# atunnd/Hair-centric-Image-Retrieval

Measured on AMD Instinct MI355X. Metric: query-images/sec (embed+top-10) ViT-B/16 vs 1M gallery, 1/2/4/8 GPU, higher is better.
Workload: dtype f16; 1 GPU; ViT-B/16 (HSimCLR ViTWrapper, random init) embed + top-10 over 1000000 x 768 f32 gallery row-sharded over 1 GPU(s); query_batch_per_gpu=880, global_query_batch=880, gallery_rows=1000000, gallery_dtype=f32, topk=10, sim_mode=filtered, residual_stream=f16, steps_in_flight=2, parallelism=gallery-shard1+query-dp1

## Files before the change

### hair-centric-image-retrieval_amd/csrc/gemm.hip

```cpp
#include "sim_core.h"
#include "act.h"
#include "gemm_plan.h"
#include "patch_plan.h"
#include "gemm_stage_addr.h"
#include <stdlib.h>

namespace {

using GemmCfg = SimCfg<_Float16, 2, 2, 2>;

constexpr int EPI_RESID_F16_STATS = 7;
constexpr int EPI_LN_BIAS_F16 = 8;
constexpr int EPI_LN_BIAS_GELU_F16 = 9;
constexpr int EPI_BIAS_F16_DUAL_GELU = 10;
constexpr int EPI_PATCH_F16_STATS = 11;

struct GemmArgs {
  const _Float16* a;
  const _Float16* w;
  const float* bias;
  const float* scale;
  void* out;
  int64_t m, lda, ldw, ldo;
  int n, k;
  const float* ln_stats;
  const float* ln_c1;
  float* stats_part;
  const void* resid;
  void* out2;
  int64_t stats_ld = 0;
};

__device__ __forceinline__ int xcd_remap(int bid, int nwg) { return gemm_xcd_remap(bid, nwg); }

template <int EPI, int NTILES>
__device__ __forceinline__ void gemm_epilogue_t(const GemmArgs& g, const f32x16 (&acc)[NTILES][2],
                                                int64_t m0, int nbase, int wave_m, int lane) {
  const int r = lane & 31, h = lane >> 5;
#pragma unroll
  for (int mt = 0; mt < 2; ++mt) {
    const int64_t m = m0 + wave_m * 64 + mt * 32 + r;
    if (m >= g.m) continue;
#pragma unroll
    for (int nt = 0; nt < NTILES; ++nt) {
#pragma unroll
      for (int grp = 0; grp < 4; ++grp) {
        const int n = nbase + nt * 32 + 8 * grp + 4 * h;
        if (n >= g.n) continue;
        f32x4 v;
#pragma unroll
        for (int e = 0; e < 4; ++e) v[e] = acc[nt][mt][4 * grp + e];
        f32x4 b = {0.f, 0.f, 0.f, 0.f};
        if (g.bias) b = *reinterpret_cast<const f32x4*>(g.bias + n);
        if constexpr (EPI == HCIR_EPI_AFFINE_RELU_F16 || EPI == HCIR_EPI_AFFINE_F32) {
          const f32x4 s = *reinterpret_cast<const f32x4*>(g.scale + n);
#pragma unroll
          for (int e = 0; e < 4; ++e) v[e] = __builtin_fmaf(v[e], s[e], b[e]);
        } else {
#pragma unroll
          for (int e = 0; e < 4; ++e) v[e] += b[e];
        }
        if constexpr (EPI == HCIR_EPI_BIAS_F16 || EPI == HCIR_EPI_BIAS_GELU_F16 ||
                      EPI == HCIR_EPI_AFFINE_RELU_F16) {
          f16x4 o;
#pragma unroll
          for (int e = 0; e < 4; ++e) {
            float x = v[e];
            if constexpr (EPI == HCIR_EPI_BIAS_GELU_F16) x = gelu_erf(x);
            if constexpr (EPI == HCIR_EPI_AFFINE_RELU_F16) x = fmaxf(x, 0.f);
            o[e] = (_Float16)x;
          }
          *reinterpret_cast<f16x4*>(static_cast<_Float16*>(g.out) + m * g.ldo + n) = o;
        } else if constexpr (EPI == HCIR_EPI_BIAS_RESID_F16) {
          _Float16* p = static_cast<_Float16*>(g.out) + m * g.ldo + n;
          const f16x4 oh = *reinterpret_cast<const f16x4*>(static_cast<const _Float16*>(g.resid) + m * g.ldo + n);
          f16x4 o;
#pragma unroll
          for (int e = 0; e < 4; ++e) {
            const float sc1 = g.scale ? g.scale[n + e] : 1.0f;
            o[e] = (_Float16)__builtin_fmaf(sc1, v[e], (float)oh[e]);
          }
          *reinterpret_cast<f16x4*>(p) = o;
        } else if constexpr (EPI == HCIR_EPI_BIAS_RESID_F32) {
          float* p = static_cast<float*>(g.out) + m * g.ldo + n;
          f32x4 o = *reinterpret_cast<const f32x4*>(static_cast<const float*>(g.resid) + m * g.ldo + n);
          if (g.scale) {
            const f32x4 s = *reinterpret_cast<const f32x4*>(g.scale + n);
#pragma unroll
            for (int e = 0; e < 4; ++e) o[e] = __builtin_fmaf(s[e], v[e], o[e]);
          } else {
#pragma unroll
            for (int e = 0; e < 4; ++e) o[e] += v[e];
          }
          *reinterpret_cast<f32x4*>(p) = o;
        } else {
          *reinterpret_cast<f32x4*>(static_cast<float*>(g.out) + m * g.ldo + n) = v;
        }
      }
    }
  }
}

template <int EPI>
__device__ __forceinline__ void gemm_epilogue(const GemmArgs& g, const f32x16 (&acc)[2][2],
                                              int64_t m0, int n0, int wave_n, int wave_m, int lane) {
  gemm_epilogue_t<EPI, 2>(g, acc, m0, n0 + wave_n * 64, wave_m, lane);
}
__device__ __forceinline__ void launder(f32x4& v) { asm volatile("" : "+v"(v)); }

struct WaveAcc {
  f32x4 a[8][4];
  __device__ __forceinline__ void zero() {
#pragma unroll
    for (int x = 0; x < 8; ++x)
#pragma unroll
      for (int y = 0; y < 4; ++y)
#pragma unroll
        for (int i = 0; i < 4; ++i) a[x][y][i] = 0.f;
  }
};

__device__ __forceinline__ float sum8_dpp(float v) {
  v += __builtin_bit_cast(float, __builtin_amdgcn_update_dpp(0, __builtin_bit_cast(int, v), 0xB1, 0xF, 0xF, true));
  v += __builtin_bit_cast(float, __builtin_amdgcn_update_dpp(0, __builtin_bit_cast(int, v), 0x4E, 0xF, 0xF, true));
  v += __builtin_bit_cast(float, __builtin_amdgcn_update_dpp(0, __builtin_bit_cast(int, v), 0x141, 0xF, 0xF, true));
  return v;
}

__device__ __forceinline__ f32x2 slice_stats8(const f16x8& o) {
  float xv[8], s1 = 0.f;
#pragma unroll
  for (int e = 0; e < 8; ++e) {
    xv[e] = (float)o[e];
    s1 += xv[e];
  }
  const float mean_s = sum8_dpp(s1) * (1.0f / 64.0f);
  float m2 = 0.f;
#pragma unroll
  for (int e = 0; e < 8; ++e) {
    const float dv = xv[e] - mean_s;
    m2 = __builtin_fmaf(dv, dv, m2);
  }
  return (f32x2){mean_s, sum8_dpp(m2)};
}

struct PatchRowMap {
  int mb, bi0, rem0, np;
  float inv;
  __device__ __forceinline__ PatchRowMap() : mb(0), bi0(0), rem0(0), np(1), inv(1.f) {}
  __device__ __forceinline__ PatchRowMap(int64_t m0w, int64_t mtot, int np_) : np(np_) {
    mb = (int)(m0w < mtot ? m0w : mtot - 1);
    bi0 = mb / np;
    rem0 = mb - bi0 * np;
    inv = 1.0f / (float)np;
  }
  __device__ __forceinline__ void map(int64_t m, int64_t mtot, int& bi, int& pi) const {
    const int r = rem0 + ((int)(m < mtot ? m : mtot - 1) - mb);
    int q = (int)((float)r * inv);
    q += ((q + 1) * np <= r) ? 1 : 0;
    q -= (q * np > r) ? 1 : 0;
    bi = bi0 + q;
    pi = r - q * np;
  }
};

template <int EPI, bool FULL, int NTW, int MTT, int MTH, class GA>
__device__ __forceinline__ void gemm_epilogue_lds_impl(const GA& g, const f32x4 (&acc)[NTW][MTT], int mt0,
                                                       char* region, int64_t m0w, int nbase, int lane) {
  constexpr bool kLn = (EPI == EPI_LN_BIAS_F16 || EPI == EPI_LN_BIAS_GELU_F16);
  constexpr bool kGelu = (EPI == HCIR_EPI_BIAS_GELU_F16 || EPI == EPI_LN_BIAS_GELU_F16);
  constexpr bool kResidH = (EPI == HCIR_EPI_BIAS_RESID_F16 || EPI == EPI_RESID_F16_STATS);
  constexpr bool kDual = (EPI == EPI_BIAS_F16_DUAL_GELU);
  constexpr bool kPatch = (EPI == EPI_PATCH_F16_STATS);
  constexpr bool kF16 = (EPI == HCIR_EPI_BIAS_F16 || kGelu || kLn ||
                         EPI == HCIR_EPI_AFFINE_RELU_F16 || kResidH || kDual || kPatch);
  constexpr bool kAffine = (EPI == HCIR_EPI_AFFINE_RELU_F16 || EPI == HCIR_EPI_AFFINE_F32);
  constexpr int FPP = kF16 ? 64 : 32;
  constexpr int NPASS = NTW * 16 / FPP;
  constexpr int NIT = MTH * 2;
  constexpr int UB = (NIT % 4 == 0) ? 4 : 3;
  static_assert(NIT % UB == 0 && (NTW * 16) % FPP == 0, "geometry");
  const int rrow = lane >> 3, rchunk = lane & 7;

  constexpr bool kScaleA = kF16 && (EPI == HCIR_EPI_AFFINE_RELU_F16 || kResidH);
  f32x4 biasA[kF16 ? NTW : 1], scaleA[kScaleA ? NTW : 1];
  bool has_scale = false;
  if constexpr (kF16) {
    has_scale = kScaleA && (EPI == HCIR_EPI_AFFINE_RELU_F16 || g.scale != nullptr);
#pragma unroll
    for (int t = 0; t < NTW; ++t) {
      const int n = nbase + 16 * t + 4 * (lane >> 4);
      biasA[t] = (f32x4){0.f, 0.f, 0.f, 0.f};
      if (g.bias) biasA[t] = *reinterpret_cast<const f32x4*>(g.bias + n);
      if constexpr (kScaleA) {
        scaleA[t] = (f32x4){1.f, 1.f, 1.f, 1.f};
        if (has_scale) scaleA[t] = *reinterpret_cast<const f32x4*>(g.scale + n);
      }
    }
  }
  constexpr int NB = kF16 ? 2 : 1;
  f32x4 bias[NPASS][NB], scale[NPASS][NB];
#pragma unroll
  for (int pass = 0; pass < NPASS; ++pass) {
    if constexpr (kF16) break;
#pragma unroll
    for (int j = 0; j < NB; ++j) {
      const int n = nbase + pass * FPP + rchunk * (kF16 ? 8 : 4) + 4 * j;
      bias[pass][j] = (f32x4){0.f, 0.f, 0.f, 0.f};
      scale[pass][j] = (f32x4){1.f, 1.f, 1.f, 1.f};
      if (g.bias) bias[pass][j] = *reinterpret_cast<const f32x4*>(g.bias + n);
      if (kAffine || (EPI == HCIR_EPI_BIAS_RESID_F32 && g.scale))
        scale[pass][j] = *reinterpret_cast<const f32x4*>(g.scale + n);
    }
  }
  float ln_rs[MTH], ln_mean[MTH];
  f32x4 c1a[NTW];
  if constexpr (kLn) {
#pragma unroll
    for (int mt = 0; mt < MTH; ++mt) {
      int64_t mm = m0w + 16 * mt + (lane & 15);
      mm = mm < g.m ? mm : g.m - 1;
      ln_mean[mt] = g.ln_stats[2 * mm];
      ln_rs[mt] = g.ln_stats[2 * mm + 1];
    }
#pragma unroll
    for (int t = 0; t < NTW; ++t) c1a[t] = *reinterpret_cast<const f32x4*>(g.ln_c1 + nbase + 16 * t + 4 * (lane >> 4));
  }
  PatchRowMap rm;
  if constexpr (kPatch) rm = PatchRowMap(m0w, g.m, g.np);
  asm volatile("s_waitcnt vmcnt(0)" ::: "memory");
  if constexpr (kLn) {
#pragma unroll
    for (int mt = 0; mt < MTH; ++mt) asm volatile("" : "+v"(ln_rs[mt]));
#pragma unroll
    for (int mt = 0; mt < MTH; ++mt) asm volatile("" : "+v"(ln_mean[mt]));
#pragma unroll
    for (int t = 0; t < NTW; ++t) launder(c1a[t]);
  }
  if constexpr (kF16) {
#pragma unroll
    for (int t = 0; t < NTW; ++t) {
      launder(biasA[t]);
      if constexpr (kScaleA) launder(scaleA[t]);
    }
  } else {
#pragma unroll
    for (int pass = 0; pass < NPASS; ++pass)
#pragma unroll
      for (int j = 0; j < NB; ++j) {
        launder(bias[pass][j]);
        launder(scale[pass][j]);
      }
  }

  constexpr int NITER = kDual ? 2 * NPASS : NPASS;
#pragma unroll
  for (int iter = 0; iter < NITER; ++iter) {
    const int pass = kDual ? iter >> 1 : iter;
    const bool second = kDual && (iter & 1);
    const int r16 = lane & 15, q16 = lane >> 4;
#pragma unroll
    for (int mt = 0; mt < MTH; ++mt) {
      const int row = mt * 16 + r16;
      if constexpr (kF16) {
        f32x4 posA[kPatch ? 4 : 1];
        if constexpr (kPatch) {
          int bi, pi;
          rm.map(m0w + row, g.m, bi, pi);
          const float* prow = g.pos + (int64_t)(1 + pi) * g.n + nbase + 64 * pass + 4 * q16;
#pragma unroll
          for (int q = 0; q < 4; ++q) posA[q] = *reinterpret_cast<const f32x4*>(prow + 16 * q);
        }
#pragma unroll
        for (int q = 0; q < 4; ++q) {
          const int nt = 4 * pass + q;
          f16x4 o;
          float xs[4];
#pragma unroll
          for (int e = 0; e < 4; ++e) {
            float x = acc[nt][mt0 + mt][e];
            const float bb = biasA[nt][e];
            if constexpr (kLn) {
              x = __builtin_fmaf(ln_rs[mt], __builtin_fmaf(-ln_mean[mt], c1a[nt][e], x), bb);
            } else if constexpr (EPI == HCIR_EPI_AFFINE_RELU_F16) {
              x = fmaxf(__builtin_fmaf(x, scaleA[nt][e], bb), 0.f);
            } else if constexpr (kResidH) {
              x = scaleA[nt][e] * (x + bb);
            } else if constexpr (kPatch) {
              x = __builtin_fmaf(g.pos_mult, posA[q][e], x + bb);
            } else {
              x += bb;
            }
            xs[e] = x;
          }
          if (kGelu || second) {
#pragma unroll
            for (int e = 0; e < 4; e += 2) {
              const gelu_f32x2 y = gelu_erf2((gelu_f32x2){xs[e], xs[e + 1]});
              xs[e] = y[0];
              xs[e + 1] = y[1];
            }
          }
#pragma unroll
          for (int e = 0; e < 4; ++e) o[e] = (_Float16)xs[e];
          const int chunk = 2 * q + (q16 >> 1);
          *reinterpret_cast<f16x4*>(region + row * 128 + ((chunk ^ (row & 7)) << 4) + 8 * (q16 & 1)) = o;
        }
      } else {
#pragma unroll
        for (int q = 0; q < 2; ++q) {
          const int nt = 2 * pass + q;
          const int chunk = 4 * q + q16;
          *reinterpret_cast<f32x4*>(region + row * 128 + ((chunk ^ (row & 7)) << 4)) = acc[nt][mt0 + mt];
        }
      }
    }
    if constexpr (kF16) {
      const int n = nbase + pass * 64 + rchunk * 8;
#pragma unroll
      for (int it0 = 0; it0 < NIT; it0 += UB) {
        f16x8 oldh[UB];
        if constexpr (kResidH) {
#pragma unroll
          for (int u = 0; u < UB; ++u) {
            const int64_t mm = m0w + (it0 + u) * 8 + rrow;
#pragma unroll
            for (int e = 0; e < 8; ++e) oldh[u][e] = (_Float16)0.f;
            if (FULL || mm < g.m)
              oldh[u] = *reinterpret_cast<const f16x8*>(static_cast<const _Float16*>(g.resid) + mm * g.ldo + n);
          }
        }
#pragma unroll
        for (int u = 0; u < UB; ++u) {
          const int row = (it0 + u) * 8 + rrow;
          const f16x8 v = *reinterpret_cast<const f16x8*>(region + row * 128 + ((rchunk ^ (row & 7)) << 4));
          f16x8 o;
          if constexpr (kResidH)
            o = v + oldh[u];
          else
            o = v;
          int64_t m = m0w + row;
          const int64_t mrow = m;
          if constexpr (kPatch) {
            int bi, pi;
            rm.map(m, g.m, bi, pi);
            m = (int64_t)bi * (g.np + 1) + 1 + pi;
          }
          if (FULL || mrow < g.m)
            __builtin_nontemporal_store(
                o, reinterpret_cast<f16x8*>(static_cast<_Float16*>(second ? g.out2 : g.out) + m * g.ldo + n));
          if constexpr (EPI == EPI_RESID_F16_STATS || kPatch) {
            const f32x2 ss = slice_stats8(o);
            if (rchunk == 0 && (FULL || mrow < g.m) && (!kPatch || g.stats_part)) {
              const int64_t slice = (nbase >> 6) + pass;
              *reinterpret_cast<f32x2*>(g.stats_part + (slice * (g.stats_ld ? g.stats_ld : g.m) + m) * 2) = ss;
            }
          }
        }
      }
    } else {
      const int n = nbase + pass * 32 + rchunk * 4;
      const f32x4 b = bias[pass][0], sc = scale[pass][0];
#pragma unroll
      for (int it0 = 0; it0 < NIT; it0 += UB) {
        f32x4 oldv[UB];
#pragma unroll
        for (int u = 0; u < UB; ++u) {
          const int64_t mm = m0w + (it0 + u) * 8 + rrow;
          oldv[u] = (f32x4){0.f, 0.f, 0.f, 0.f};
          if constexpr (EPI == HCIR_EPI_BIAS_RESID_F32) {
            if (FULL || mm < g.m)
              oldv[u] = *reinterpret_cast<const f32x4*>(static_cast<const float*>(g.resid) + mm * g.ldo + n);
          }
        }
#pragma unroll
        for (int u = 0; u < UB; ++u) {
          const int row = (it0 + u) * 8 + rrow;
          const int64_t mm = m0w + row;
          f32x4 v = *reinterpret_cast<const f32x4*>(region + row * 128 + ((rchunk ^ (row & 7)) << 4));
          if constexpr (EPI == HCIR_EPI_AFFINE_F32) {
#pragma unroll
            for (int e = 0; e < 4; ++e) v[e] = __builtin_fmaf(v[e], sc[e], b[e]);
          } else if constexpr (EPI == HCIR_EPI_BIAS_RESID_F32) {
#pragma unroll
            for (int e = 0; e < 4; ++e) v[e] = __builtin_fmaf(sc[e], v[e] + b[e], oldv[u][e]);
          } else {
#pragma unroll
            for (int e = 0; e < 4; ++e) v[e] += b[e];
          }
          if (FULL || mm < g.m) *reinterpret_cast<f32x4*>(static_cast<float*>(g.out) + mm * g.ldo + n) = v;
        }
      }
    }
  }
}

template <int EPI, int NTW, int MTT, int MTH, class GA>
__device__ __forceinline__ void gemm_epilogue_lds(const GA& g, const f32x4 (&acc)[NTW][MTT], int mt0,
                                                  char* region, int64_t m0w, int nbase, int lane) {
  asm volatile("" : "+v"(lane));
  if (m0w + 16 * MTH <= g.m)
    gemm_epilogue_lds_impl<EPI, true, NTW, MTT, MTH>(g, acc, mt0, region, m0w, nbase, lane);
  else
    gemm_epilogue_lds_impl<EPI, false, NTW, MTT, MTH>(g, acc, mt0, region, m0w, nbase, lane);
}

template <int EPI, bool GLDS>
__global__ __launch_bounds__(256, 2) void gemm_f16_kernel(GemmArgs g, int tiles_n, int tiles_m) {
  using Cfg = GemmCfg;
  __shared__ __attribute__((aligned(16))) char lds[Cfg::LDS_BYTES];
  const int tid = threadIdx.x, lane = tid & 63, wave = tid >> 6;
  const int wave_n = wave >> 1, wave_m = wave & 1;
  const int t = xcd_remap(blockIdx.x, tiles_n * tiles_m);
  const int tn = t % tiles_n, tm = t / tiles_n;
  const int n0 = tn * 128;
  const int64_t m0 = (int64_t)tm * 128;
  const int nkc = (g.k + 63) / 64;

  f32x16 acc[2][2];
#pragma unroll
  for (int a = 0; a < 2; ++a)
#pragma unroll
    for (int b = 0; b < 2; ++b)
#pragma unroll
      for (int i = 0; i < 16; ++i) acc[a][b][i] = 0.f;

  if constexpr (GLDS) {
    sim_stage_glds<_Float16, Cfg>(lds, g.w, n0, g.n - 1, g.a, m0, g.m - 1, g.k, 0, tid);
    for (int kc = 0; kc < nkc; ++kc) {
      const int cur = kc & 1;
      sim_glds_retire_and_sync();
      if (kc + 1 < nkc)
        sim_stage_glds<_Float16, Cfg>(lds + (cur ^ 1) * Cfg::STAGE_BYTES, g.w, n0, g.n - 1, g.a, m0,
                                      g.m - 1, g.k, kc + 1, tid);
      sim_stage_mfma<_Float16, Cfg, 2>(acc, lds + cur * Cfg::STAGE_BYTES, wave_n, wave_m, lane);
    }
  } else {
    u32x4 regs[Cfg::NLOAD];
    sim_stage_load<_Float16, Cfg>(regs, g.w, n0, g.n - 1, g.a, m0, g.m - 1, g.k, 0, tid);
    sim_stage_store<Cfg>(regs, lds, tid);
    __syncthreads();
    for (int kc = 0; kc < nkc; ++kc) {
      const int cur = kc & 1;
      if (kc + 1 < nkc)
        sim_stage_load<_Float16, Cfg>(regs, g.w, n0, g.n - 1, g.a, m0, g.m - 1, g.k, kc + 1, tid);
      sim_stage_mfma<_Float16, Cfg, 2>(acc, lds + cur * Cfg::STAGE_BYTES, wave_n, wave_m, lane);
      if (kc + 1 < nkc) sim_stage_store<Cfg>(regs, lds + (cur ^ 1) * Cfg::STAGE_BYTES, tid);
      __syncthreads();
    }
  }
  gemm_epilogue<EPI>(g, acc, m0, n0, wave_n, wave_m, lane);
}

#ifdef HCIR_DIAG_GSTAMPS
__device__ unsigned long long g_gemm_stamps[256 * 8];
#define HCIR_GSTAMP(cond, i)                                                                   \
  do {                                                                                         \
    if ((cond) && threadIdx.x == 0 && blockIdx.x < 256)                                        \
      g_gemm_stamps[blockIdx.x * 8 + (i)] = __builtin_amdgcn_s_memrealtime();                  \
  } while (0)
#else
#define HCIR_GSTAMP(cond, i) \
  do {                       \
  } while (0)
#endif


struct G256 {
  static constexpr int NT = 512;
  static constexpr int TN = 256, TM = 256;
  static constexpr int WAVES_N = 2, WAVES_M = 4;
  static constexpr int ROWS = TN + TM;
  static constexpr int STAGE_BYTES = ROWS * 128;
  static constexpr int NLOAD = ROWS * 8 / NT;
  static constexpr int NW = TN * 8 / NT;
  static constexpr bool N_GROUPED = true;
  static_assert(WAVES_N * WAVES_M * 64 == NT && NT * NW == TN * 8, "geometry");
};

struct GMid {
  static constexpr int NT = 256;
  static constexpr int TN = 128, TM = 192;
  static constexpr int WAVES_N = 2, WAVES_M = 2;
  static constexpr int ROWS = TN + TM;
  static constexpr int STAGE_BYTES = ROWS * 128;
  static constexpr int NLOAD = ROWS * 8 / NT;
  static constexpr int NW = TN * 8 / NT;
  static constexpr bool N_GROUPED = false;
  static_assert(WAVES_N * WAVES_M * 64 == NT && NT * NW == TN * 8, "geometry");
};

template <class G>
struct GemmStages {
  int issue_kc = 0, issue_ti = 0;
  const char* wbase = nullptr;
  const char* abase = nullptr;
  int a_last = 0;
  GemmTileOrigins org;
  const GemmArgs& g;
  char* const lds;
  const int tiles_n, tiles_m, tid;
  const int ntiles = tiles_n * tiles_m;
  const int nkc = g.k / 64;
  const int my_tiles =
      (int)blockIdx.x < ntiles ? (ntiles - (int)blockIdx.x + (int)gridDim.x - 1) / (int)gridDim.x : 0;
  const int nsteps = my_tiles * nkc;
  const int wave_dst = __builtin_amdgcn_readfirstlane((tid & ~63) * 16);
  uint32_t woff, aoff;

  __device__ __forceinline__ GemmStages(const GemmArgs& g_, char* lds_, int tiles_n_, int tiles_m_, int tid_)
      : g(g_), lds(lds_), tiles_n(tiles_n_), tiles_m(tiles_m_), tid(tid_) {
    set_lane_offsets();
  }

  __device__ __forceinline__ void set_lane_offsets() {
    int otid = tid;
    asm volatile("" : "+v"(otid));
    woff = gemm_lane_off(otid, g.ldw);
    aoff = gemm_lane_off(otid, g.lda);
  }

  __device__ __forceinline__ void tile_origin(int ti, int& n0, int64_t& m0) const {
    gemm_tile_origin<G::N_GROUPED, G::TN, G::TM>((int)blockIdx.x, (int)gridDim.x, ti, tiles_n, tiles_m, n0, m0);
  }

  __device__ __forceinline__ void origin(int ti, int& n0, int64_t& m0) const {
    int mt;
    org.get(issue_ti - ti, n0, mt);
    m0 = (int64_t)mt * G::TM;
  }

  __device__ __forceinline__ void next_tile() {
    org.shift();
    if (issue_ti < my_tiles) {
      int n0;
      int64_t m0;
      tile_origin(issue_ti, n0, m0);
      org.set(n0, (int)(m0 / G::TM));
      wbase = reinterpret_cast<const char*>(g.w + (int64_t)n0 * g.ldw);
      abase = reinterpret_cast<const char*>(g.a + m0 * g.lda);
      a_last = gemm_tile_last_row<G::TM>(g.m, m0);
    }
  }

  __device__ __forceinline__ bool ragged() const { return a_last < G::TM - 1; }

  template <bool RAGGED>
  __device__ __forceinline__ void issue_piece_as(int slot, int i) const {
    const uint32_t dst = lds_addr(lds) + slot * G::STAGE_BYTES + wave_dst + G::NT * i * 16;
    int otid = tid;
    if constexpr (RAGGED) asm volatile("" : "+v"(otid));
    int64_t base;
    uint32_t off;
// ... 376 lines not shown
    const int bfirst = (int)m0 / g.np;
    ibase = reinterpret_cast<const char*>(g.img + (int64_t)bfirst * g.c * g.h * g.w_px);
#pragma unroll
    for (int i = 0; i < NA; ++i) {
      int64_t m = m0 + (otid >> 3) + 64 * i;
      m = m < g.m ? m : g.m - 1;
      const int mi = (int)m;
      const int bi = mi / g.np, pi = mi - bi * g.np;
      const int py = pi / g.gw, px = pi - py * g.gw;
      aoff[i] = (uint32_t)((((bi - bfirst) * g.c * g.h + py * 16 + (chunk >> 1)) * g.w_px + px * 16 + 8 * (chunk & 1)) * 4);
    }
  };
  f32x4 stage_a[2 * NA];
  auto gather_load = [&](int kc) {
    const char* kbase = ibase + ((int64_t)(kc >> 2) * g.h + 4 * (kc & 3)) * g.w_px * 4;
#pragma unroll
    for (int i = 0; i < NA; ++i) {
      stage_a[2 * i] = *reinterpret_cast<const f32x4*>(kbase + aoff[i]);
      stage_a[2 * i + 1] = *reinterpret_cast<const f32x4*>(kbase + aoff[i] + 16);
    }
  };
  auto gather_store = [&](int slot) {
#pragma unroll
    for (int i = 0; i < NA; ++i) {
      f16x8 v;
#pragma unroll
      for (int e = 0; e < 4; ++e) {
        v[e] = (_Float16)stage_a[2 * i][e];
        v[4 + e] = (_Float16)stage_a[2 * i + 1][e];
      }
      *reinterpret_cast<f16x8*>(lds + slot * G256::STAGE_BYTES + sim_slot_off(G256::TN + (tid >> 3) + 64 * i, tid & 7)) = v;
    }
  };

  WaveAcc acc;
  acc.zero();

  if (nsteps > 0) {
    stg.next_tile();
    set_rows(0);
    gather_load(0);
#pragma unroll
    for (int i = 0; i < G256::NW; ++i) stg.issue_piece(0, i);
    gather_store(0);
    stg.issue_advance();
    if (stg.issue_kc == 0 && stg.issue_ti < stg.my_tiles) set_rows(stg.issue_ti);
  }

  int kc = 0, ti = 0;
  for (int step = 0; step < nsteps; ++step) {
    asm volatile("s_waitcnt vmcnt(0) lgkmcnt(0)" ::: "memory");
    __builtin_amdgcn_s_barrier();

    const char* st = lds + (step & 1) * G256::STAGE_BYTES;
    const bool do_issue = step + 1 < nsteps;
    const int islot = (step + 1) & 1;
    const int r16 = lane & 15, kq = lane >> 4;
    if (do_issue) gather_load(stg.issue_kc);
#pragma unroll
    for (int ks2 = 0; ks2 < 2; ++ks2) {
      const int chunk = 4 * ks2 + kq;
      u32x4 bf[4];
#pragma unroll
      for (int mt = 0; mt < 4; ++mt)
        bf[mt] = *reinterpret_cast<const u32x4*>(st + sim_slot_off(G256::TN + wave_m * 64 + mt * 16 + r16, chunk));
#pragma unroll
      for (int half = 0; half < 2; ++half) {
        u32x4 af[4];
#pragma unroll
        for (int q = 0; q < 4; ++q)
          af[q] = *reinterpret_cast<const u32x4*>(
              st + sim_slot_off(wave_n * 128 + (4 * half + q) * 16 + r16, chunk));
        if (do_issue && ks2 == 0 && half == 0) {
#pragma unroll
          for (int i = 0; i < G256::NW; ++i) stg.issue_piece(islot, i);
        }
#pragma unroll
        for (int q = 0; q < 4; ++q)
#pragma unroll
          for (int mt = 0; mt < 4; ++mt)
            acc.a[4 * half + q][mt] = __builtin_amdgcn_mfma_f32_16x16x32_f16(
                __builtin_bit_cast(f16x8, af[q]), __builtin_bit_cast(f16x8, bf[mt]), acc.a[4 * half + q][mt],
                0, 0, 0);
      }
    }
    if (do_issue) {
      gather_store(islot);
      stg.issue_advance();
      if (stg.issue_kc == 0 && stg.issue_ti < stg.my_tiles) set_rows(stg.issue_ti);
    }

    if (++kc == nkc) {
      int n0;
      int64_t m0;
      stg.tile_origin(ti, n0, m0);
      __builtin_amdgcn_s_barrier();
      gemm_epilogue_lds<EPI_PATCH_F16_STATS, 8, 4, 4>(g, acc.a, 0, lds + (step & 1) * G256::STAGE_BYTES + wave * 8192,
                                                      m0 + wave_m * 64, n0 + wave_n * 128, lane);
      acc.zero();
      kc = 0;
      ++ti;
      if (stg.issue_ti < stg.my_tiles) set_rows(stg.issue_ti);
    }
  }
}

__global__ __launch_bounds__(256) void cls_row_stats_kernel(const float* __restrict__ cls, const float* __restrict__ pos,
                                                            float pos_mult, int64_t b, int t, int d,
                                                            _Float16* __restrict__ tok, float* __restrict__ stats_part) {
  const int per = d >> 3;
  const int64_t total = b * per;
  int64_t i = (int64_t)blockIdx.x * blockDim.x + threadIdx.x;
  const bool inside = i < total;
  i = inside ? i : total - 1;
  const int64_t bi = i / per;
  const int n = (int)(i - bi * per) * 8;
  f16x8 o;
#pragma unroll
  for (int j = 0; j < 2; ++j) {
    const f32x4 cv = *reinterpret_cast<const f32x4*>(cls + n + 4 * j);
    const f32x4 pv = *reinterpret_cast<const f32x4*>(pos + n + 4 * j);
#pragma unroll
    for (int e = 0; e < 4; ++e) o[4 * j + e] = (_Float16)__builtin_fmaf(pos_mult, pv[e], cv[e]);
  }
  const f32x2 ss = slice_stats8(o);
  if (!inside) return;
  const int64_t row = bi * t;
  *reinterpret_cast<f16x8*>(tok + row * d + n) = o;
  if (stats_part && (threadIdx.x & 7) == 0)
    *reinterpret_cast<f32x2*>(stats_part + ((int64_t)(n >> 6) * (b * t) + row) * 2) = ss;
}

__global__ void ln_stats_finalize_kernel(const float* __restrict__ part, int parts, int64_t m, float slice_n,
                                         float eps, float* __restrict__ stats) {
  const int64_t row = (int64_t)blockIdx.x * blockDim.x + threadIdx.x;
  if (row >= m) return;
  float ms = 0.f;
  for (int p = 0; p < parts; ++p) ms += part[((int64_t)p * m + row) * 2];
  const float mean = ms / (float)parts;
  float m2 = 0.f;
  for (int p = 0; p < parts; ++p) {
    const f32x2 v = *reinterpret_cast<const f32x2*>(part + ((int64_t)p * m + row) * 2);
    const float dm = v[0] - mean;
    m2 += v[1] + slice_n * dm * dm;
  }
  const float var = m2 / (slice_n * (float)parts);
  *reinterpret_cast<f32x2*>(stats + 2 * row) = (f32x2){mean, 1.0f / sqrtf(var + eps)};
}

template <int EPI>
void launch_gemm_mid(const GemmArgs& g, hipStream_t st) {
  const int tn = g.n / GMid::TN, tm = (int)hcir_cdiv(g.m, GMid::TM);
  const int grid = tn * tm < 512 ? tn * tm : 512;
  hipLaunchKernelGGL((gemm_f16_mid_kernel<EPI>), dim3(grid), dim3(GMid::NT), 0, st, g, tn, tm);
}

template <int EPI>
void launch_big_tiles(const GemmArgs& g, int tn, int tm, hipStream_t st) {
  const int grid = tn * tm < 256 ? tn * tm : 256;
  hipLaunchKernelGGL((gemm_f16_big_kernel<EPI>), dim3(grid), dim3(G256::NT), 0, st, g, tn, tm);
}

template <int EPI>
void launch_gemm_big(const GemmArgs& g, const GemmPlan& p, hipStream_t st) {
  if constexpr (EPI != EPI_BIAS_F16_DUAL_GELU) {
    if (p.route == HCIR_GEMM_ROUTE_SPLIT) {
      const int64_t m1 = p.m1;
      GemmArgs g1 = g, g2 = g;
      g1.m = m1;
      g1.stats_ld = g.stats_ld ? g.stats_ld : g.m;
      g2.m = g.m - m1;
      g2.stats_ld = g1.stats_ld;
      g2.a = g.a + m1 * g.lda;
      const bool f32out = EPI == HCIR_EPI_BIAS_RESID_F32 || EPI == HCIR_EPI_BIAS_F32 || EPI == HCIR_EPI_AFFINE_F32;
      const int64_t obytes = m1 * g.ldo * (f32out ? 4 : 2);
      g2.out = static_cast<char*>(g.out) + obytes;
      if (g.resid) g2.resid = static_cast<const char*>(g.resid) + obytes;
      if (g.ln_stats) g2.ln_stats = g.ln_stats + 2 * m1;
      if (g.stats_part) g2.stats_part = g.stats_part + 2 * m1;
      launch_big_tiles<EPI>(g1, p.tn, p.tm1, st);
      launch_gemm_mid<EPI>(g2, st);
      return;
    }
    if (p.route == HCIR_GEMM_ROUTE_MID) {
      launch_gemm_mid<EPI>(g, st);
      return;
    }
  }
  launch_big_tiles<EPI>(g, p.tn, p.tm, st);
}

template <int EPI>
void launch_gemm(const GemmArgs& g, hipStream_t st) {
  const GemmPlan p = gemm_plan(g.m, g.n, g.k, EPI == EPI_BIAS_F16_DUAL_GELU);
  if (p.route != HCIR_GEMM_ROUTE_SMALL) {
    launch_gemm_big<EPI>(g, p, st);
    return;
  }
  if (g.k % 64 == 0)
    hipLaunchKernelGGL((gemm_f16_kernel<EPI, true>), dim3(p.tn * p.tm), dim3(256), 0, st, g, p.tn, p.tm);
  else
    hipLaunchKernelGGL((gemm_f16_kernel<EPI, false>), dim3(p.tn * p.tm), dim3(256), 0, st, g, p.tn, p.tm);
}

}

extern "C" {

int hcir_gemm_f16(const void* a, int64_t lda, const void* w, int64_t ldw, const float* bias,
                  const float* scale, int64_t m, int32_t n, int32_t k, int epilogue, void* out,
                  int64_t ldo, void* stream) {
  return hcir_gemm_f16_resid(a, lda, w, ldw, bias, scale, m, n, k, epilogue, nullptr, out, ldo, stream);
}

int hcir_gemm_f16_resid(const void* a, int64_t lda, const void* w, int64_t ldw, const float* bias,
                        const float* scale, int64_t m, int32_t n, int32_t k, int epilogue, const void* resid,
                        void* out, int64_t ldo, void* stream) {
  HCIR_ENTER();
  if (resid && epilogue != HCIR_EPI_BIAS_RESID_F16 && epilogue != HCIR_EPI_BIAS_RESID_F32) return HCIR_ERR_INVALID;
  if (!a || !w || !out || m <= 0 || n <= 0 || k <= 0) return HCIR_ERR_INVALID;
  if ((k & 7) || (n & 7) || lda < k || ldw < k || (lda & 7) || (ldw & 7) || ldo < n || (ldo & 3))
    return HCIR_ERR_INVALID;
  const bool f16out = epilogue == HCIR_EPI_BIAS_F16 || epilogue == HCIR_EPI_BIAS_GELU_F16 ||
                      epilogue == HCIR_EPI_AFFINE_RELU_F16 || epilogue == HCIR_EPI_BIAS_RESID_F16;
  if (f16out && gemm_takes_big(m, n, k) && (ldo & 7)) return HCIR_ERR_INVALID;
  if ((lda != k || ldw != k) && !gemm_takes_big(m, n, k)) return HCIR_ERR_UNSUPPORTED;
  if ((epilogue == HCIR_EPI_AFFINE_RELU_F16 || epilogue == HCIR_EPI_AFFINE_F32) && !scale)
    return HCIR_ERR_INVALID;
  if (hcir_cdiv(m, 128) * hcir_cdiv(n, 128) > 0x7fffffff) return HCIR_ERR_INVALID;
  GemmArgs g{static_cast<const _Float16*>(a), static_cast<const _Float16*>(w), bias, scale, out, m,
             lda, ldw, ldo, n, k, nullptr, nullptr, nullptr, resid ? resid : out, nullptr};
  hipStream_t st = static_cast<hipStream_t>(stream);
  switch (epilogue) {
    case HCIR_EPI_BIAS_F16: launch_gemm<HCIR_EPI_BIAS_F16>(g, st); break;
    case HCIR_EPI_BIAS_GELU_F16: launch_gemm<HCIR_EPI_BIAS_GELU_F16>(g, st); break;
    case HCIR_EPI_BIAS_RESID_F32: launch_gemm<HCIR_EPI_BIAS_RESID_F32>(g, st); break;
    case HCIR_EPI_BIAS_F32: launch_gemm<HCIR_EPI_BIAS_F32>(g, st); break;
    case HCIR_EPI_AFFINE_RELU_F16: launch_gemm<HCIR_EPI_AFFINE_RELU_F16>(g, st); break;
    case HCIR_EPI_AFFINE_F32: launch_gemm<HCIR_EPI_AFFINE_F32>(g, st); break;
    case HCIR_EPI_BIAS_RESID_F16: launch_gemm<HCIR_EPI_BIAS_RESID_F16>(g, st); break;
    default: return HCIR_ERR_UNSUPPORTED;
  }
  HCIR_LAUNCH_CHECK();
  return HCIR_OK;
}

int hcir_gemm_f16_gelu_dual(const void* a, int64_t lda, const void* w, int64_t ldw, const float* bias, int64_t m,
                            int32_t n, int32_t k, void* out_pre, void* out_act, int64_t ldo, void* stream) {
  HCIR_ENTER();
  if (!a || !w || !out_pre || !out_act || m <= 0 || n <= 0 || k <= 0) return HCIR_ERR_INVALID;
  if (lda < k || ldw < k || (lda & 7) || (ldw & 7) || ldo < n || (ldo & 7)) return HCIR_ERR_INVALID;
  if (!gemm_takes_big(m, n, k)) return HCIR_ERR_UNSUPPORTED;
  GemmArgs g{static_cast<const _Float16*>(a), static_cast<const _Float16*>(w), bias, nullptr, out_pre, m,
             lda, ldw, ldo, n, k, nullptr, nullptr, nullptr, out_pre, out_act};
  launch_gemm_big<EPI_BIAS_F16_DUAL_GELU>(g, gemm_plan(m, n, k, true), static_cast<hipStream_t>(stream));
  HCIR_LAUNCH_CHECK();
  return HCIR_OK;
}

#ifdef HCIR_DIAG_GSTAMPS
int hcir_debug_gemm_stamps(unsigned long long* host_dst) {
  return (int)hipMemcpyFromSymbol(host_dst, HIP_SYMBOL(g_gemm_stamps), sizeof(unsigned long long) * 256 * 8);
}
#endif

int hcir_gemm_fused_supported(int64_t m, int32_t n, int32_t k) { return gemm_takes_big(m, n, k) ? 1 : 0; }

int32_t hcir_gemm_stats_slices(int32_t n) { return n / 64; }

int hcir_gemm_route(int64_t m, int32_t n, int32_t k, int epilogue, int64_t* rows_on_big) {
  if (m <= 0 || n <= 0 || k <= 0 || (k & 7) || (n & 7)) return HCIR_ERR_INVALID;
  if (epilogue < HCIR_EPI_BIAS_F16 || (epilogue > HCIR_EPI_BIAS_RESID_F16 && epilogue != HCIR_GEMM_ROUTE_EPI_DUAL))
    return HCIR_ERR_INVALID;
  const GemmPlan p = gemm_plan(m, n, k, epilogue == HCIR_GEMM_ROUTE_EPI_DUAL);
  if (rows_on_big) *rows_on_big = p.m1;
  return p.route;
}

int hcir_gemm_f16_fused(const void* a, int64_t lda, const void* w, int64_t ldw, const float* bias,
                        const float* scale, int64_t m, int32_t n, int32_t k, int epilogue, void* out,
                        int64_t ldo, const float* ln_stats, const float* ln_c1, float* stats_part,
                        void* stream) {
  HCIR_ENTER();
  if (!a || !w || !out || m <= 0 || n <= 0 || k <= 0) return HCIR_ERR_INVALID;
  if ((k & 7) || (n & 7) || lda < k || ldw < k || (lda & 7) || (ldw & 7) || ldo < n || (ldo & 7))
    return HCIR_ERR_INVALID;
  const bool ln = ln_stats || ln_c1;
  if (ln && (!ln_stats || !ln_c1 || !bias)) return HCIR_ERR_INVALID;
  if (ln && stats_part) return HCIR_ERR_INVALID;
  if (!ln && !stats_part) return HCIR_ERR_INVALID;
  if (ln && epilogue != HCIR_EPI_BIAS_F16 && epilogue != HCIR_EPI_BIAS_GELU_F16) return HCIR_ERR_UNSUPPORTED;
  if (stats_part && epilogue != HCIR_EPI_BIAS_RESID_F16) return HCIR_ERR_UNSUPPORTED;
  if (!gemm_takes_big(m, n, k)) return HCIR_ERR_UNSUPPORTED;
  GemmArgs g{static_cast<const _Float16*>(a), static_cast<const _Float16*>(w), bias, scale, out, m,
             lda, ldw, ldo, n, k, ln_stats, ln_c1, stats_part, out, nullptr};
  hipStream_t st = static_cast<hipStream_t>(stream);
  const GemmPlan p = gemm_plan(m, n, k, false);
  if (stats_part) launch_gemm_big<EPI_RESID_F16_STATS>(g, p, st);
  else if (epilogue == HCIR_EPI_BIAS_F16) launch_gemm_big<EPI_LN_BIAS_F16>(g, p, st);
  else launch_gemm_big<EPI_LN_BIAS_GELU_F16>(g, p, st);
  HCIR_LAUNCH_CHECK();
  return HCIR_OK;
}

int hcir_gemm_f16_ln_rows(const void* a, int64_t lda, const void* w, int64_t ldw, const float* bias, int64_t m,
                          int32_t n, int32_t k, void* out, int64_t ldo, const float* ln_stats, const float* ln_c1,
                          void* stream) {
  HCIR_ENTER();
  if (!a || !w || !out || !bias || !ln_stats || !ln_c1 || m <= 0 || n <= 0 || k <= 0) return HCIR_ERR_INVALID;
  if (lda < k || ldw < k || (lda & 7) || (ldw & 7) || ldo < n || (ldo & 7)) return HCIR_ERR_INVALID;
  if (k % 64 || n % GMid::TN) return HCIR_ERR_UNSUPPORTED;
  if ((n / GMid::TN) * hcir_cdiv(m, GMid::TM) > 0x7fffffff) return HCIR_ERR_INVALID;
  GemmArgs g{static_cast<const _Float16*>(a), static_cast<const _Float16*>(w), bias, nullptr, out, m,
// ... 104 lines not shown
```

Before: 26810 query-images/sec.

## Scalarize GEMM epilogue row addressing and specialize layer-scale residual epilogue

Reworks the LDS-staged GEMM epilogue so global row addresses are computed once per block in scalar registers and advanced by a fixed group step, with a per-lane 32-bit offset replacing per-row 64-bit multiply-adds. Residual epilogues gain separate template variants with and without layer-scale, chosen at launch by whether a scale pointer is set, so the common path skips loading the scale vector and the multiply. Stats writes are batched after the stores, and wave-uniform m0w/nbase are forced to SGPRs via readfirstlane. The aim is lower VALU and VGPR pressure in the epilogue, at the cost of more kernel instantiations and reliance on 32-bit lane offsets fitting.

```diff
diff --git a/hair-centric-image-retrieval_amd/csrc/gemm.hip b/hair-centric-image-retrieval_amd/csrc/gemm.hip
--- a/hair-centric-image-retrieval_amd/csrc/gemm.hip
+++ b/hair-centric-image-retrieval_amd/csrc/gemm.hip
@@ -3,6 +3,7 @@
 #include "gemm_plan.h"
 #include "patch_plan.h"
 #include "gemm_stage_addr.h"
+#include "gemm_epilogue_rows.h"
 #include <stdlib.h>
 
 namespace {
@@ -14,6 +15,11 @@
 constexpr int EPI_LN_BIAS_GELU_F16 = 9;
 constexpr int EPI_BIAS_F16_DUAL_GELU = 10;
 constexpr int EPI_PATCH_F16_STATS = 11;
+constexpr int EPI_RESID_F16_SCALE = 12;
+constexpr int EPI_RESID_F16_STATS_SCALE = 13;
+constexpr int epi_with_scale(int epi) {
+  return epi == HCIR_EPI_BIAS_RESID_F16 ? EPI_RESID_F16_SCALE : epi == EPI_RESID_F16_STATS ? EPI_RESID_F16_STATS_SCALE : epi;
+}
 
 struct GemmArgs {
   const _Float16* a;
@@ -114,9 +120,12 @@
 #pragma unroll
     for (int x = 0; x < 8; ++x)
 #pragma unroll
-      for (int y = 0; y < 4; ++y)
-#pragma unroll
-        for (int i = 0; i < 4; ++i) a[x][y][i] = 0.f;
+      for (int y = 0; y < 4; ++y) {
+        f32x2 lo, hi;
+        asm volatile("v_mov_b64 %0, 0" : "=v"(lo));
+        asm volatile("v_mov_b64 %0, 0" : "=v"(hi));
+        a[x][y] = (f32x4){lo[0], lo[1], hi[0], hi[1]};
+      }
   }
 };
 
@@ -169,7 +178,9 @@
                                                        char* region, int64_t m0w, int nbase, int lane) {
   constexpr bool kLn = (EPI == EPI_LN_BIAS_F16 || EPI == EPI_LN_BIAS_GELU_F16);
   constexpr bool kGelu = (EPI == HCIR_EPI_BIAS_GELU_F16 || EPI == EPI_LN_BIAS_GELU_F16);
-  constexpr bool kResidH = (EPI == HCIR_EPI_BIAS_RESID_F16 || EPI == EPI_RESID_F16_STATS);
+  constexpr bool kStats = (EPI == EPI_RESID_F16_STATS || EPI == EPI_RESID_F16_STATS_SCALE);
+  constexpr bool kLayerScale = (EPI == EPI_RESID_F16_SCALE || EPI == EPI_RESID_F16_STATS_SCALE);
+  constexpr bool kResidH = (EPI == HCIR_EPI_BIAS_RESID_F16 || kStats || kLayerScale);
   constexpr bool kDual = (EPI == EPI_BIAS_F16_DUAL_GELU);
   constexpr bool kPatch = (EPI == EPI_PATCH_F16_STATS);
   constexpr bool kF16 = (EPI == HCIR_EPI_BIAS_F16 || kGelu || kLn ||
@@ -182,20 +193,15 @@
   static_assert(NIT % UB == 0 && (NTW * 16) % FPP == 0, "geometry");
   const int rrow = lane >> 3, rchunk = lane & 7;
 
-  constexpr bool kScaleA = kF16 && (EPI == HCIR_EPI_AFFINE_RELU_F16 || kResidH);
+  constexpr bool kScaleA = kF16 && (EPI == HCIR_EPI_AFFINE_RELU_F16 || kLayerScale);
   f32x4 biasA[kF16 ? NTW : 1], scaleA[kScaleA ? NTW : 1];
-  bool has_scale = false;
   if constexpr (kF16) {
-    has_scale = kScaleA && (EPI == HCIR_EPI_AFFINE_RELU_F16 || g.scale != nullptr);
 #pragma unroll
     for (int t = 0; t < NTW; ++t) {
       const int n = nbase + 16 * t + 4 * (lane >> 4);
       biasA[t] = (f32x4){0.f, 0.f, 0.f, 0.f};
       if (g.bias) biasA[t] = *reinterpret_cast<const f32x4*>(g.bias + n);
-      if constexpr (kScaleA) {
-        scaleA[t] = (f32x4){1.f, 1.f, 1.f, 1.f};
-        if (has_scale) scaleA[t] = *reinterpret_cast<const f32x4*>(g.scale + n);
-      }
+      if constexpr (kScaleA) scaleA[t] = *reinterpret_cast<const f32x4*>(g.scale + n);
     }
   }
   constexpr int NB = kF16 ? 2 : 1;
@@ -252,6 +258,26 @@
         launder(scale[pass][j]);
       }
   }
+
+  constexpr bool kScalarRows = !kPatch && !kDual;
+  constexpr int ES = kF16 ? 2 : 4;
+  const int64_t row_base = gemm_epi_block_base(m0w, g.ldo, nbase, ES), row_step = gemm_epi_group_step(g.ldo, ES);
+  const int rows_left = FULL ? 16 * MTH : gemm_epi_rows_left(g.m, m0w, 16 * MTH);
+  uint32_t row_lane = gemm_epi_lane_off(lane, g.ldo, ES);
+  const char* rd = region + gemm_epi_lds_lane_off(lane);
+  using gchar = __attribute__((address_space(1))) char;
+  using gf16x8 = __attribute__((address_space(1))) f16x8;
+  using gf32x4 = __attribute__((address_space(1))) f32x4;
+  auto row_at = [&](gchar* at, int pass, uint32_t lane_off) { return at + pass * 128 + lane_off; };
+  auto first_group = [&](const void* buf) {
+    gchar* at = (gchar*)(static_cast<const char*>(buf) + row_base);
+    if constexpr (kScalarRows) asm volatile("" : "+s"(at));
+    return at;
+  };
+  auto next_group = [&](gchar*& at) {
+    at += row_step;
+    if constexpr (kScalarRows) asm("" : "+s"(at));
+  };
 
   constexpr int NITER = kDual ? 2 * NPASS : NPASS;
 #pragma unroll
@@ -285,7 +311,8 @@
             } else if constexpr (EPI == HCIR_EPI_AFFINE_RELU_F16) {
               x = fmaxf(__builtin_fmaf(x, scaleA[nt][e], bb), 0.f);
             } else if constexpr (kResidH) {
-              x = scaleA[nt][e] * (x + bb);
+              x += bb;
+              if constexpr (kLayerScale) x = scaleA[nt][e] * x;
             } else if constexpr (kPatch) {
               x = __builtin_fmaf(g.pos_mult, posA[q][e], x + bb);
             } else {
@@ -315,69 +342,87 @@
         }
       }
     }
+    gchar* ld_at = (kResidH || EPI == HCIR_EPI_BIAS_RESID_F32) ? first_group(g.resid) : nullptr;
+    gchar* st_at = first_group(second ? g.out2 : g.out);
     if constexpr (kF16) {
       const int n = nbase + pass * 64 + rchunk * 8;
+      char* const stats_base =
+          kStats
+              ? reinterpret_cast<char*>(g.stats_part) +
+                    gemm_epi_stats_base((nbase >> 6) + pass, g.stats_ld ? g.stats_ld : g.m, m0w) +
+                    gemm_epi_stats_lane_off(lane)
+              : nullptr;
 #pragma unroll
       for (int it0 = 0; it0 < NIT; it0 += UB) {
+        uint32_t rl = row_lane;
+        if constexpr (kStats) asm volatile("" : "+v"(rl));
         f16x8 oldh[UB];
         if constexpr (kResidH) {
 #pragma unroll
           for (int u = 0; u < UB; ++u) {
-            const int64_t mm = m0w + (it0 + u) * 8 + rrow;
 #pragma unroll
             for (int e = 0; e < 8; ++e) oldh[u][e] = (_Float16)0.f;
-            if (FULL || mm < g.m)
-              oldh[u] = *reinterpret_cast<const f16x8*>(static_cast<const _Float16*>(g.resid) + mm * g.ldo + n);
+            if (FULL || gemm_epi_row_ok(lane, it0 + u, rows_left))
+              oldh[u] = *reinterpret_cast<const gf16x8*>(row_at(ld_at, pass, rl));
+            next_group(ld_at);
           }
         }
+        f32x2 ss[UB];
+        int64_t mtok[UB];
 #pragma unroll
         for (int u = 0; u < UB; ++u) {
-          const int row = (it0 + u) * 8 + rrow;
-          const f16x8 v = *reinterpret_cast<const f16x8*>(region + row * 128 + ((rchunk ^ (row & 7)) << 4));
+          const f16x8 v = *reinterpret_cast<const f16x8*>(rd + (it0 + u) * kGemmEpiLdsGroupStep);
           f16x8 o;
           if constexpr (kResidH)
             o = v + oldh[u];
           else
             o = v;
-          int64_t m = m0w + row;
-          const int64_t mrow = m;
+          gf16x8* dst;
           if constexpr (kPatch) {
             int bi, pi;
-            rm.map(m, g.m, bi, pi);
-            m = (int64_t)bi * (g.np + 1) + 1 + pi;
+            rm.map(m0w + (it0 + u) * 8 + rrow, g.m, bi, pi);
+            mtok[u] = (int64_t)bi * (g.np + 1) + 1 + pi;
+            dst = (gf16x8*)(static_cast<_Float16*>(g.out) + mtok[u] * g.ldo + n);
+          } else {
+            dst = reinterpret_cast<gf16x8*>(row_at(st_at, pass, rl));
           }
-          if (FULL || mrow < g.m)
-            __builtin_nontemporal_store(
-                o, reinterpret_cast<f16x8*>(static_cast<_Float16*>(second ? g.out2 : g.out) + m * g.ldo + n));
-          if constexpr (EPI == EPI_RESID_F16_STATS || kPatch) {
-            const f32x2 ss = slice_stats8(o);
-            if (rchunk == 0 && (FULL || mrow < g.m) && (!kPatch || g.stats_part)) {
-              const int64_t slice = (nbase >> 6) + pass;
-              *reinterpret_cast<f32x2*>(g.stats_part + (slice * (g.stats_ld ? g.stats_ld : g.m) + m) * 2) = ss;
+          if (FULL || gemm_epi_row_ok(lane, it0 + u, rows_left)) __builtin_nontemporal_store(o, dst);
+          next_group(st_at);
+          if constexpr (kStats || kPatch) ss[u] = slice_stats8(o);
+        }
+        if constexpr (kStats || kPatch) {
+          if (rchunk == 0 && (!kPatch || g.stats_part)) {
+#pragma unroll
+            for (int u = 0; u < UB; ++u) {
+              if (FULL || gemm_epi_row_ok(lane, it0 + u, rows_left)) {
+                if constexpr (kPatch) {
+                  const int64_t slice = (nbase >> 6) + pass;
+                  *reinterpret_cast<f32x2*>(g.stats_part + (slice * (g.stats_ld ? g.stats_ld : g.m) + mtok[u]) * 2) = ss[u];
+                } else {
+                  *reinterpret_cast<f32x2*>(stats_base + (it0 + u) * kGemmEpiStatsGroupStep) = ss[u];
+                }
+              }
             }
           }
         }
       }
     } else {
-      const int n = nbase + pass * 32 + rchunk * 4;
       const f32x4 b = bias[pass][0], sc = scale[pass][0];
 #pragma unroll
       for (int it0 = 0; it0 < NIT; it0 += UB) {
         f32x4 oldv[UB];
 #pragma unroll
         for (int u = 0; u < UB; ++u) {
-          const int64_t mm = m0w + (it0 + u) * 8 + rrow;
           oldv[u] = (f32x4){0.f, 0.f, 0.f, 0.f};
           if constexpr (EPI == HCIR_EPI_BIAS_RESID_F32) {
-            if (FULL || mm < g.m)
-              oldv[u] = *reinterpret_cast<const f32x4*>(static_cast<const float*>(g.resid) + mm * g.ldo + n);
+            if (FULL || gemm_epi_row_ok(lane, it0 + u, rows_left))
+              oldv[u] = *reinterpret_cast<const gf32x4*>(row_at(ld_at, pass, row_lane));
+            next_group(ld_at);
           }
         }
 #pragma unroll
         for (int u = 0; u < UB; ++u) {
-          const int row = (it0 + u) * 8 + rrow;
-          const int64_t mm = m0w + row;
-          f32x4 v = *reinterpret_cast<const f32x4*>(region + row * 128 + ((rchunk ^ (row & 7)) << 4));
+          f32x4 v = *reinterpret_cast<const f32x4*>(rd + (it0 + u) * kGemmEpiLdsGroupStep);
           if constexpr (EPI == HCIR_EPI_AFFINE_F32) {
 #pragma unroll
             for (int e = 0; e < 4; ++e) v[e] = __builtin_fmaf(v[e], sc[e], b[e]);
@@ -388,7 +433,9 @@
 #pragma unroll
             for (int e = 0; e < 4; ++e) v[e] += b[e];
           }
-          if (FULL || mm < g.m) *reinterpret_cast<f32x4*>(static_cast<float*>(g.out) + mm * g.ldo + n) = v;
+          if (FULL || gemm_epi_row_ok(lane, it0 + u, rows_left))
+            *reinterpret_cast<gf32x4*>(row_at(st_at, pass, row_lane)) = v;
+          next_group(st_at);
         }
       }
     }
@@ -399,6 +446,11 @@
 __device__ __forceinline__ void gemm_epilogue_lds(const GA& g, const f32x4 (&acc)[NTW][MTT], int mt0,
                                                   char* region, int64_t m0w, int nbase, int lane) {
   asm volatile("" : "+v"(lane));
+  if constexpr (EPI != EPI_PATCH_F16_STATS && EPI != EPI_BIAS_F16_DUAL_GELU) {
+    m0w = (int64_t)(((uint64_t)(uint32_t)__builtin_amdgcn_readfirstlane((int)(m0w >> 32)) << 32) |
+                    (uint32_t)__builtin_amdgcn_readfirstlane((int)m0w));
+    nbase = __builtin_amdgcn_readfirstlane(nbase);
+  }
   if (m0w + 16 * MTH <= g.m)
     gemm_epilogue_lds_impl<EPI, true, NTW, MTT, MTH>(g, acc, mt0, region, m0w, nbase, lane);
   else
@@ -1081,13 +1133,19 @@
 void launch_gemm_mid(const GemmArgs& g, hipStream_t st) {
   const int tn = g.n / GMid::TN, tm = (int)hcir_cdiv(g.m, GMid::TM);
   const int grid = tn * tm < 512 ? tn * tm : 512;
-  hipLaunchKernelGGL((gemm_f16_mid_kernel<EPI>), dim3(grid), dim3(GMid::NT), 0, st, g, tn, tm);
+  if (epi_with_scale(EPI) != EPI && g.scale)
+    hipLaunchKernelGGL((gemm_f16_mid_kernel<epi_with_scale(EPI)>), dim3(grid), dim3(GMid::NT), 0, st, g, tn, tm);
+  else
+    hipLaunchKernelGGL((gemm_f16_mid_kernel<EPI>), dim3(grid), dim3(GMid::NT), 0, st, g, tn, tm);
 }
 
 template <int EPI>
 void launch_big_tiles(const GemmArgs& g, int tn, int tm, hipStream_t st) {
   const int grid = tn * tm < 256 ? tn * tm : 256;
-  hipLaunchKernelGGL((gemm_f16_big_kernel<EPI>), dim3(grid), dim3(G256::NT), 0, st, g, tn, tm);
+  if (epi_with_scale(EPI) != EPI && g.scale)
+    hipLaunchKernelGGL((gemm_f16_big_kernel<epi_with_scale(EPI)>), dim3(grid), dim3(G256::NT), 0, st, g, tn, tm);
+  else
+    hipLaunchKernelGGL((gemm_f16_big_kernel<EPI>), dim3(grid), dim3(G256::NT), 0, st, g, tn, tm);
 }
 
 template <int EPI>
diff --git a/hair-centric-image-retrieval_amd/csrc/gemm_epilogue_rows.h b/hair-centric-image-retrieval_amd/csrc/gemm_epilogue_rows.h
--- /dev/null
+++ b/hair-centric-image-retrieval_amd/csrc/gemm_epilogue_rows.h
@@ -0,0 +1,34 @@
+#pragma once
+#include <stdint.h>
+
+#if defined(__HIPCC__)
+#define GEMM_EPI_FN __host__ __device__ __forceinline__
+#else
+#define GEMM_EPI_FN static inline
+#endif
+
+GEMM_EPI_FN int64_t gemm_epi_block_base(int64_t m0w, int64_t ld, int nbase, int esize) {
+  return (m0w * ld + nbase) * esize;
+}
+
+GEMM_EPI_FN int64_t gemm_epi_group_step(int64_t ld, int esize) { return 8 * ld * esize; }
+
+GEMM_EPI_FN uint32_t gemm_epi_lane_off(int lane, int64_t ld, int esize) {
+  return ((uint32_t)(lane >> 3) * (uint32_t)ld + (uint32_t)(lane & 7) * (uint32_t)(16 / esize)) * (uint32_t)esize;
+}
+
+GEMM_EPI_FN int64_t gemm_epi_stats_base(int64_t slice, int64_t rows, int64_t m0w) { return (slice * rows + m0w) * 8; }
+GEMM_EPI_FN uint32_t gemm_epi_stats_lane_off(int lane) { return (uint32_t)(lane >> 3) * 8u; }
+constexpr int kGemmEpiStatsGroupStep = 64;
+
+GEMM_EPI_FN uint32_t gemm_epi_lds_lane_off(int lane) {
+  return (uint32_t)(lane >> 3) * 128u + (uint32_t)(((lane & 7) ^ (lane >> 3)) << 4);
+}
+constexpr int kGemmEpiLdsGroupStep = 1024;
+
+GEMM_EPI_FN int gemm_epi_rows_left(int64_t m, int64_t m0w, int rows) {
+  const int64_t left = m - m0w;
+  return left <= 0 ? 0 : (left < rows ? (int)left : rows);
+}
+
+GEMM_EPI_FN bool gemm_epi_row_ok(int lane, int it, int rows_left) { return it * 8 + (lane >> 3) < rows_left; }
```

Result: no change. 26920 query-images/sec, median of 6 (+0.4%).
